# mitiko/weath3rb0i

Hardware: AMD Instinct MI355X
Metric: encode MiB/s, 64 KiB blocks, bit-exact vs CPU ref (higher is better)
Workload: dtype u32

## Files before the change

include/w3hip.h:

```cpp
#ifndef W3HIP_H
#define W3HIP_H

#include <stddef.h>
#include <stdint.h>

#ifdef __cplusplus
extern "C" {
#endif

#define W3_ABI_VERSION 8

enum {
    W3_OK            =  0,
    W3_E_INVALID     = -1,
    W3_E_NOSPACE     = -2,
    W3_E_HIP         = -3,
    W3_E_UNSUPPORTED = -4,
    W3_E_NOMEM       = -5,
    W3_E_FORMAT      = -6,
    W3_E_CORRUPT     = -7
};

enum { W3_NODE_ORDERN = 1, W3_NODE_BEST_OF_TWO = 2, W3_NODE_SLOT_STATE = 3, W3_NODE_APM = 4 };
enum { W3_HIST_NONE = 0, W3_HIST_RAW = 1, W3_HIST_AC = 2, W3_HIST_HUFF = 3 };
// ... 202 lines not shown
                       const uint8_t *in, size_t n, uint8_t *out, size_t out_cap, size_t *out_len);
int w3_decompress_stream(w3_ctx *ctx, const w3_model_spec *spec,
                         const uint8_t *in, size_t in_len, uint8_t *out, size_t out_cap, size_t *out_len);

int w3_predict_blocks(w3_ctx *ctx, const w3_model_spec *spec,
                      const uint8_t *in, size_t n, size_t block_size, uint16_t *p_out);

int w3_stationary_table(const uint8_t *buf, size_t n, uint16_t table[8]);

int w3_huff_tables(const uint8_t *buf, size_t n, uint8_t huff_size, uint8_t rem_huff_size, w3_huff_table *out);

#define W3_STAT_TILE 4096u
#define W3_STAT_BATCH 64u
#define W3_HIST_REP 16u
typedef struct w3_prep_profile {
    float hist_ms, hist_sum_ms, stat_count_ms, stat_walk_ms;
    uint32_t halvings[8];
    uint16_t table[8];
    uint64_t counts[256];
} w3_prep_profile;
int w3_histogram(w3_ctx *ctx, const uint8_t *in, size_t n, uint64_t counts[256]);
int w3_histogram_device(w3_ctx *ctx, const uint8_t *d_in, size_t n, uint64_t counts[256] , void *stream);
int w3_stationary_table_staged(w3_ctx *ctx, const uint8_t *in, size_t n, uint16_t table[8]);
int w3_stationary_table_device(w3_ctx *ctx, const uint8_t *d_in, size_t n, uint16_t table[8] , void *stream);
int w3_huff_code_from_counts(const uint64_t counts[256], uint8_t huffman_size, w3_huff_code *out);
int w3_huff_tables_from_counts(const uint64_t counts[256], uint8_t huff_size, uint8_t rem_huff_size, w3_huff_table *out);
int w3_table_prep_profile(w3_ctx *ctx, const uint8_t *d_in, size_t n, uint32_t hist_rep, w3_prep_profile *out);

#define W3_STATE_TABLE_SIZE 3963
int w3_state_table(uint16_t *out );
int w3_stretch_squash(int16_t *stretch , uint16_t *squash );

int w3_selftest_counter_p(w3_ctx *ctx, uint64_t *mismatches);

int w3_debug_get_stamps(w3_ctx *ctx, uint64_t out[8]);

typedef struct w3_timing {
    float    predict_ms;
    float    coder_ms;
    float    pack_ms;
    float    generic_ms;
    float    total_ms;
    uint32_t path;
    uint32_t n_coder_launches;
    uint64_t coder_bytes;
    uint64_t predict_bytes;
    uint32_t n_recoded_blocks;
    float    apm_ms;
    float    slot_ms;
    uint32_t n_slot_launches;
    float    achash_ms;
    uint32_t n_parts;
    uint32_t n_lds_faults;
    uint32_t n_wide;
    float    part_ms[4];
    float    rank_ms[4];
    float    small_ms;
} w3_timing;
int w3_get_timing(const w3_ctx *ctx, w3_timing *out);

#ifdef __cplusplus
}
#endif
#endif
```

weath3rb0i_amd/_lib.py:

```python
import ctypes as C
import os

HERE = os.path.dirname(os.path.abspath(__file__))
SO = os.environ.get("W3HIP_SO") or os.path.join(HERE, "libw3hip.so")

W3_MAX_NODES = 31
W3_NODE_ORDERN, W3_NODE_BEST_OF_TWO, W3_NODE_SLOT_STATE, W3_NODE_APM = 1, 2, 3, 4
W3_APM_ORDER0, W3_APM_ORDER1 = 0, 1
W3_MAX_APM = 4
W3_HIST_NONE, W3_HIST_RAW, W3_HIST_AC, W3_HIST_HUFF = 0, 1, 2, 3
W3_MAX_HUFF = 4
W3_OK, W3_E_INVALID, W3_E_NOSPACE, W3_E_HIP, W3_E_UNSUPPORTED, W3_E_NOMEM, W3_E_FORMAT = 0, -1, -2, -3, -4, -5, -6
W3_E_CORRUPT = -7
W3_OPT_PATH, W3_OPT_TIMING, W3_OPT_CODER, W3_OPT_ACC_LIMIT, W3_OPT_DEBUG_STAMPS, W3_OPT_VARIANT, W3_OPT_SLOT_BUDGET_MB, W3_OPT_VERIFY, W3_OPT_FAULT_BLOCK, W3_OPT_TUNE, W3_OPT_HOST_CHUNK_BLOCKS, W3_OPT_FAULT_KERNELS, W3_OPT_AOH_BATCH_BLOCKS = 1, 2, 3, 4, 5, 7, 8, 9, 10, 11, 12, 13, 14
W3_OPT_EXPORT_EPOCH = 15
W3_VAR_NO_LDS_ATOMICS, W3_VAR_PARTITION4, W3_VAR_NO_CHAINED_PARTITION, W3_VAR_CM_UNSTAGED, W3_VAR_NO_SIDE_STREAM, W3_VAR_INJECT_LDS_FAULT = 1, 2, 4, 8, 16, 32
W3_VAR_HALF_CU, W3_VAR_FULL_CU = 64, 128
W3_VAR_SLOT_TABLE, W3_VAR_SLOT_SORTED, W3_VAR_DECODE_LANE, W3_VAR_AOH_DECODE_SPEC = 256, 512, 1024, 2048
W3_GATHER_AUTO, W3_GATHER_RCCL, W3_GATHER_PEER_COPY = 0, 1, 2
W3_PATH_AUTO, W3_PATH_GENERIC, W3_PATH_TWOPHASE, W3_PATH_SPEC = 0, 1, 2, 3


class Node(C.Structure):
    _fields_ = [("kind", C.c_uint8), ("bits", C.c_uint8), ("align", C.c_uint8), ("history", C.c_uint8),
# ... 19 lines not shown
class Check(C.Structure):
    _fields_ = [("crc", C.c_void_p), ("bad_block", C.c_uint64), ("n_bad", C.c_uint64)]


class Timing(C.Structure):
    _fields_ = [("predict_ms", C.c_float), ("coder_ms", C.c_float), ("pack_ms", C.c_float), ("generic_ms", C.c_float),
                ("total_ms", C.c_float), ("path", C.c_uint32), ("n_coder_launches", C.c_uint32),
                ("coder_bytes", C.c_uint64), ("predict_bytes", C.c_uint64), ("n_recoded_blocks", C.c_uint32), ("apm_ms", C.c_float),
                ("slot_ms", C.c_float), ("n_slot_launches", C.c_uint32), ("achash_ms", C.c_float), ("n_parts", C.c_uint32),
                ("n_lds_faults", C.c_uint32), ("n_wide", C.c_uint32), ("part_ms", C.c_float * 4), ("rank_ms", C.c_float * 4),
                ("small_ms", C.c_float)]


class PrepProfile(C.Structure):
    _fields_ = [("hist_ms", C.c_float), ("hist_sum_ms", C.c_float), ("stat_count_ms", C.c_float), ("stat_walk_ms", C.c_float),
                ("halvings", C.c_uint32 * 8), ("table", C.c_uint16 * 8), ("counts", C.c_uint64 * 256)]


class ExportProfile(C.Structure):
    _fields_ = [("epochs", C.c_uint64), ("replays", C.c_uint64), ("halvings", C.c_uint64),
                ("count_ms", C.c_float), ("apply_ms", C.c_float), ("replay_ms", C.c_float), ("total_ms", C.c_float)]


class ExportEntropyProfile(C.Structure):
    _fields_ = [("base", ExportProfile), ("key_ms", C.c_float), ("huff_fixed_epochs", C.c_uint64)]


W3_STAT_TILE, W3_STAT_BATCH, W3_HIST_REP = 4096, 64, 16

EXPORTS = [
    "w3_abi_version", "w3_strerror", "w3_last_error", "w3_ctx_create", "w3_ctx_destroy", "w3_spec_validate",
    "w3_ctx_set_option", "w3_max_compressed_size", "w3_encode_blocks", "w3_decode_blocks", "w3_encode_blocks_device",
    "w3_decode_blocks_device", "w3_encode_submit", "w3_encode_wait", "w3_encode_max_in_flight", "w3_compress_stream", "w3_decompress_stream", "w3_predict_blocks", "w3_stationary_table",
    "w3_get_timing", "w3_selftest_counter_p", "w3_debug_get_stamps", "w3_state_table", "w3_stretch_squash", "w3_huff_tables",
    "w3_shard_range", "w3_encode_blocks_sharded", "w3_encode_blocks_sharded_device", "w3_encode_stats", "w3_encode_stats_device", "w3_sweep_ordern", "w3_sweep_ordern_device", "w3_export_counters",
    "w3_encode_host_submit", "w3_encode_host_wait", "w3_encode_host_max_in_flight", "w3_rccl_library", "w3_rccl_status",
    "w3_encode_sharded_submit", "w3_encode_sharded_wait", "w3_encode_sharded_max_in_flight",
    "w3_decode_ranges", "w3_decode_ranges_device",
    "w3_huff_code_table", "w3_aoh_max_compressed_size", "w3_aoh_encode_blocks", "w3_aoh_encode_blocks_device", "w3_aoh_decode_blocks",
    "w3_aoh_decode_blocks_device", "w3_aoh_encode_stats", "w3_aoh_encode_stats_device", "w3_sweep_ac_over_huffman",
    "w3_sweep_ac_over_huffman_device", "w3_aoh_decode_ranges", "w3_aoh_decode_ranges_device", "w3_aoh_decode_spec_covers",
    "w3_crc32_blocks", "w3_crc32_blocks_device", "w3_crc32_verify_device", "w3_decode_blocks_checked", "w3_decode_ranges_checked",
    "w3_decode_ranges_device_checked", "w3_aoh_decode_blocks_checked", "w3_aoh_decode_ranges_checked", "w3_aoh_decode_ranges_device_checked",
    "w3_histogram", "w3_histogram_device", "w3_stationary_table_staged", "w3_stationary_table_device", "w3_huff_code_from_counts",
    "w3_huff_tables_from_counts", "w3_table_prep_profile",
    "w3_export_counters_device", "w3_export_counters_staged", "w3_export_get_profile",
    "w3_export_entropy_device", "w3_export_entropy_staged", "w3_export_entropy_get_profile",
]

_lib = None


def load():
    global _lib
    if _lib is not None:
        return _lib
    if not os.path.exists(SO):
        raise ImportError(
            "weath3rb0i_amd: HIP extension %s is missing - run `python -m weath3rb0i_amd.build` "
            "(or __graft_entry__.build()).  There is no CPU fallback." % SO)
    try:
        import torch
    except ImportError:
        pass
    lib = C.CDLL(SO)
    vp, sz = C.c_void_p, C.c_size_t
    lib.w3_abi_version.restype = C.c_int
    lib.w3_strerror.restype = C.c_char_p
    lib.w3_strerror.argtypes = [C.c_int]
    lib.w3_last_error.restype = C.c_char_p
    lib.w3_last_error.argtypes = [vp]
    lib.w3_ctx_create.argtypes = [C.c_int, C.POINTER(vp)]
    lib.w3_ctx_destroy.argtypes = [vp]
    lib.w3_ctx_destroy.restype = None
    lib.w3_spec_validate.argtypes = [C.POINTER(ModelSpec)]
    lib.w3_ctx_set_option.argtypes = [vp, C.c_int, C.c_int64]
    lib.w3_max_compressed_size.restype = sz
    lib.w3_max_compressed_size.argtypes = [sz, sz]
    lib.w3_encode_blocks.argtypes = [vp, C.POINTER(ModelSpec), vp, sz, sz, vp, sz, C.POINTER(sz), vp]
    lib.w3_decode_blocks.argtypes = [vp, C.POINTER(ModelSpec), vp, sz, vp, sz, sz, C.c_uint64, vp]
    lib.w3_encode_blocks_device.argtypes = [vp, C.POINTER(ModelSpec), vp, sz, sz, vp, sz, vp, vp, vp]
    lib.w3_decode_blocks_device.argtypes = [vp, C.POINTER(ModelSpec), vp, sz, vp, sz, sz, C.c_uint64, vp, vp]
    lib.w3_encode_submit.argtypes = [vp, C.POINTER(ModelSpec), vp, sz, sz, vp, sz, vp, vp, vp, C.POINTER(C.c_int)]
    lib.w3_encode_wait.argtypes = [vp, C.c_int]
    lib.w3_encode_max_in_flight.argtypes = [C.POINTER(ModelSpec), sz, sz]
    lib.w3_encode_max_in_flight.restype = C.c_int
    lib.w3_compress_stream.argtypes = [vp, C.POINTER(ModelSpec), vp, sz, vp, sz, C.POINTER(sz)]
    lib.w3_decompress_stream.argtypes = [vp, C.POINTER(ModelSpec), vp, sz, vp, sz, C.POINTER(sz)]
    lib.w3_predict_blocks.argtypes = [vp, C.POINTER(ModelSpec), vp, sz, sz, vp]
    lib.w3_stationary_table.argtypes = [vp, sz, vp]
    lib.w3_selftest_counter_p.argtypes = [vp, C.POINTER(C.c_uint64)]
    lib.w3_debug_get_stamps.argtypes = [vp, C.POINTER(C.c_uint64 * 8)]
    lib.w3_get_timing.argtypes = [vp, C.POINTER(Timing)]
    lib.w3_state_table.argtypes = [vp]
    lib.w3_stretch_squash.argtypes = [vp, vp]
    lib.w3_huff_tables.argtypes = [vp, sz, C.c_uint8, C.c_uint8, C.POINTER(HuffTable)]
    lib.w3_shard_range.argtypes = [sz, C.c_int, C.c_int, C.POINTER(sz), C.POINTER(sz)]
    lib.w3_encode_blocks_sharded.argtypes = [C.POINTER(vp), C.c_int, C.POINTER(ModelSpec), vp, sz, sz, vp, sz, C.POINTER(sz), vp]
    lib.w3_encode_blocks_sharded_device.argtypes = [C.POINTER(vp), C.c_int, C.POINTER(ModelSpec), C.POINTER(vp), C.POINTER(sz), sz, C.c_int, vp, sz, vp,
                                                    C.POINTER(C.c_uint64), C.c_int]
    lib.w3_encode_stats.argtypes = [vp, C.POINTER(ModelSpec), vp, sz, sz, vp]
    lib.w3_encode_stats_device.argtypes = [vp, C.POINTER(ModelSpec), vp, sz, sz, vp, vp]
    lib.w3_sweep_ordern.argtypes = [vp, vp, sz, sz, vp, vp, sz, vp]
    lib.w3_sweep_ordern_device.argtypes = [vp, vp, sz, sz, vp, vp, sz, vp]
    lib.w3_export_counters.argtypes = [vp, C.POINTER(ModelSpec), vp, sz, vp]
    lib.w3_encode_host_submit.argtypes = [vp, C.POINTER(ModelSpec), vp, sz, sz, vp, sz, vp, C.POINTER(C.c_int)]
    lib.w3_encode_host_wait.argtypes = [vp, C.c_int, C.POINTER(sz)]
    lib.w3_encode_host_max_in_flight.argtypes = [C.POINTER(ModelSpec), sz, sz]
    lib.w3_encode_host_max_in_flight.restype = C.c_int
    lib.w3_encode_sharded_submit.argtypes = [C.POINTER(vp), C.c_int, C.POINTER(ModelSpec), C.POINTER(vp), C.POINTER(sz), sz, C.POINTER(C.c_int)]
    lib.w3_encode_sharded_wait.argtypes = [C.POINTER(vp), C.c_int, C.c_int, C.c_int, vp, sz, vp, C.POINTER(C.c_uint64), C.c_int]
    lib.w3_encode_sharded_max_in_flight.argtypes = [C.POINTER(ModelSpec), C.POINTER(sz), C.c_int, sz]
    lib.w3_encode_sharded_max_in_flight.restype = C.c_int
    lib.w3_decode_ranges.argtypes = [vp, C.POINTER(ModelSpec), vp, sz, vp, sz, sz, C.c_uint64, C.POINTER(Range), sz, vp, sz, C.POINTER(sz)]
    lib.w3_decode_ranges_device.argtypes = [vp, C.POINTER(ModelSpec), vp, sz, vp, sz, sz, C.c_uint64, C.POINTER(Range), sz, vp, sz, C.POINTER(sz), vp]
    hc, u8 = C.POINTER(HuffCode), C.c_uint8
    lib.w3_huff_code_table.argtypes = [vp, sz, u8, hc]
    lib.w3_aoh_max_compressed_size.restype = sz
    lib.w3_aoh_max_compressed_size.argtypes = [sz, sz, hc]
    lib.w3_aoh_encode_blocks.argtypes = [vp, hc, u8, vp, sz, sz, vp, sz, C.POINTER(sz), vp]
    lib.w3_aoh_encode_blocks_device.argtypes = [vp, hc, u8, vp, sz, sz, vp, sz, vp, vp, vp]
    lib.w3_aoh_decode_blocks.argtypes = [vp, hc, u8, vp, sz, vp, sz, sz, C.c_uint64, vp]
    lib.w3_aoh_decode_blocks_device.argtypes = [vp, hc, u8, vp, sz, vp, sz, sz, C.c_uint64, vp, vp]
    lib.w3_aoh_decode_ranges.argtypes = [vp, hc, u8, vp, sz, vp, sz, sz, C.c_uint64, C.POINTER(Range), sz, vp, sz, C.POINTER(sz)]
# ... 35 lines not shown
```

weath3rb0i_amd/csrc/w3_device.h:

```cpp
#pragma once
#include <hip/hip_runtime.h>
#include <stdint.h>

namespace w3 {

__device__ __forceinline__ uint32_t counter_p(uint32_t c0, uint32_t c1) {
    const uint32_t d = c0 + c1 + 2u;
    const uint32_t a = c1 + 1u;
    const float t = (float)a * __builtin_amdgcn_rcpf((float)d);
    uint32_t p = (uint32_t)__builtin_fmaf(t, 65536.0f, 0.47f);
    const uint32_t d2 = d + d;
    const uint32_t R = ((a << 17) + d) - __umul24(p, d2);
    return p + (R >= d2 ? 1u : 0u);
}

__device__ __forceinline__ uint32_t counter_p_packed(uint32_t c) { return counter_p(c & 0xFFFFu, c >> 16); }

__device__ __forceinline__ uint32_t counter_update_packed(uint32_t c, uint32_t bit) {
    uint32_t c0 = c & 0xFFFFu, c1 = c >> 16;
    if (bit) c1 += 1u; else c0 += 1u;
    if ((bit ? c1 : c0) == 0xFFFFu) {
        c0 = (c0 >> 1) + (c0 & 1u);
        c1 = (c1 >> 1) + (c1 & 1u);
    }
    return c0 | (c1 << 16);
}

__device__ __forceinline__ uint32_t opinion_dist(uint32_t p) { return p >= 32768u ? p - 32768u : 32768u - p; }
typedef unsigned short u16x2 __attribute__((ext_vector_type(2)));
typedef short i16x2 __attribute__((ext_vector_type(2)));
__device__ __forceinline__ u16x2 as_u16x2(uint32_t v) { return __builtin_bit_cast(u16x2, v); }
__device__ __forceinline__ i16x2 as_i16x2(u16x2 v) { return __builtin_bit_cast(i16x2, v); }
__device__ __forceinline__ uint32_t as_u32(u16x2 v) { return __builtin_bit_cast(uint32_t, v); }
__device__ __forceinline__ uint32_t as_u32(i16x2 v) { return __builtin_bit_cast(uint32_t, v); }
__device__ __forceinline__ u16x2 pk_opinion_dist(u16x2 p) {
    const u16x2 half = {32768, 32768};
    return __builtin_elementwise_max(p, half) - __builtin_elementwise_min(p, half);
}
__device__ __forceinline__ uint32_t pk_farther_mask(u16x2 d, u16x2 e) {
    uint32_t m;
    asm("v_pk_sub_i16 %0, %1, %2\n\tv_pk_ashrrev_i16 %0, 15, %0 op_sel_hi:[0,1]" : "=&v"(m) : "v"(as_u32(d)), "v"(as_u32(e)));
    return m;
}


struct BitSink {
    uint64_t acc;
    uint32_t nb;
    uint8_t *base;
// ... 237 lines not shown
```

weath3rb0i_amd/csrc/w3_predict.h:

```cpp
#pragma once
#include "w3_device.h"
#include "../../include/w3hip.h"

namespace w3 {

#define W3_PF 8

#define W3_HALF_CU_LDS 81920u
template <int NW, size_t USED> struct HalfCuPad { static constexpr size_t words = (NW > 1 && USED < W3_HALF_CU_LDS) ? (W3_HALF_CU_LDS - USED + 3u) / 4u : (NW > 1 ? 0u : 1u); };
template <size_t WORDS> struct HalfCuPadDecl {
    static __device__ __forceinline__ void keep(uint64_t n) {
        __shared__ uint32_t pad_[WORDS];
        if (n == ~0ull) pad_[threadIdx.x % WORDS] = 1u;
    }
};
template <> struct HalfCuPadDecl<0> { static __device__ __forceinline__ void keep(uint64_t) {} };
#define W3_HALF_CU_PAD(NW, USED) HalfCuPadDecl<((NW) > 1 ? HalfCuPad<NW, (USED)>::words : 0u)>::keep(a.n);

struct PredictArgs {
    const uint8_t *in;
    uint64_t n;
    uint32_t block_size, nblocks;
    uint4 *P;
    const uint2 *keys;
// ... 51 lines not shown
#pragma unroll
        for (int j = 0; j < 8; j++) {
            uint64_t m = ~0ull;
#pragma unroll
            for (int k = 0; k < H; k++) m &= X[8 - j + k];
            M[j] = m;
        }
    }
}

template <int H>
__device__ __forceinline__ void match_keys(uint2 k8, uint64_t M[8]) {
#pragma unroll
    for (int j = 0; j < 8; j++) {
        const uint32_t key = ((j < 4 ? k8.x : k8.y) >> (8 * (j & 3))) & 0xFFu;
        uint32_t mlo = 0xFFFFFFFFu, mhi = 0xFFFFFFFFu;
#pragma unroll
        for (int k = 0; k < H; k++) {
            const uint32_t sm = (uint32_t)__builtin_amdgcn_sbfe((int)key, k, 1);
            const uint64_t B = __ballot(sm != 0u);
            mlo &= ~((uint32_t)B ^ sm);
            mhi &= ~((uint32_t)(B >> 32) ^ sm);
        }
        M[j] = ((uint64_t)mhi << 32) | mlo;
    }
}

__device__ __forceinline__ uint32_t mbcnt64(uint64_t m) {
    return __builtin_amdgcn_mbcnt_hi((uint32_t)(m >> 32), __builtin_amdgcn_mbcnt_lo((uint32_t)m, 0u));
}

template <bool GROUPED>
__device__ __forceinline__ void rank_round(uint32_t c0, const uint32_t key[8], const uint64_t M[8], uint64_t seg, bool valid, bool rd,
                                           uint32_t *tbl, uint32_t p[8], uint32_t fin[8], uint32_t &wmask) {
    __asm__ volatile("" ::: "memory");
    const uint64_t gt = lane_gt_mask();
    const int lane = threadIdx.x & 63;
    wmask = 0u;
    uint32_t basev[8];
#pragma unroll
    for (int j = 0; j < 8; j++) basev[j] = tbl[j * 256 + key[j]];
#pragma unroll
    for (int j = 0; j < 8; j++) {
        const uint64_t Mj = M[j] & seg;
        const uint32_t bit = (c0 >> (7 - j)) & 1u;
        const uint64_t ones = __ballot(bit) & Mj;
        uint32_t base = basev[j];
        if constexpr (GROUPED) base = rd ? base : 0u;
        const uint32_t b0 = base & 0xFFFFu, b1 = base >> 16;
        const uint32_t n1l = mbcnt64(ones), n0l = mbcnt64(Mj) - n1l;
        uint32_t s0 = b0 + n0l, s1 = b1 + n1l;
        const bool last = valid && (Mj & gt) == 0ull;
        uint32_t f0 = s0 + (bit ^ 1u), f1 = s1 + bit;
        uint64_t satm = __ballot(last && (f0 >= 65535u || f1 >= 65535u));
        uint32_t f = f0 | (f1 << 16);
        while (satm) {
            const int k = __ffsll((long long)satm) - 1;
            const uint64_t Mc = readlane_u64(Mj, k);
            const uint64_t Oc = readlane_u64(ones, k);
            uint32_t st = readlane_u32(base, k);
            uint64_t it = Mc;
            while (it) {
                const int m = __ffsll((long long)it) - 1;
                it &= it - 1;
                if (lane == m) { s0 = st & 0xFFFFu; s1 = st >> 16; }
                st = counter_update_packed(st, (uint32_t)(Oc >> m) & 1u);
            }
            if (lane == k) f = st;
            satm &= satm - 1;
        }
        p[j] = counter_p(s0, s1);
        fin[j] = f;
        wmask |= last ? (1u << j) : 0u;
    }
    if constexpr (!GROUPED) {
#pragma unroll
        for (int j = 0; j < 8; j++)
            if ((wmask >> j) & 1u) tbl[j * 256 + key[j]] = fin[j];
        __asm__ volatile("" ::: "memory");
    }
}

#define W3_ATOMIC_LIM 65400u
#ifndef W3_ATOMIC_MAXSEG
#define W3_ATOMIC_MAXSEG 4u
#endif
typedef uint16_t w3_u16x2 __attribute__((ext_vector_type(2)));

__device__ __forceinline__ void atomic_round(uint32_t *tbl, uint32_t c0, const uint32_t key[8], bool on, uint32_t v[8]) {
#pragma unroll
    for (int j = 0; j < 8; j++) {
        const uint32_t inc = on ? (((c0 >> (7 - j)) & 1u) ? 0x10000u : 1u) : 0u;
        v[j] = __hip_atomic_fetch_add(&tbl[j * 256 + key[j]], inc, __ATOMIC_RELAXED, __HIP_MEMORY_SCOPE_WORKGROUP);
    }
}
__device__ __forceinline__ bool atomic_round_hot(const uint32_t v[8]) {
    w3_u16x2 m = __builtin_bit_cast(w3_u16x2, v[0]);
#pragma unroll
    for (int j = 1; j < 8; j++) m = __builtin_elementwise_max(m, __builtin_bit_cast(w3_u16x2, v[j]));
    return __ballot(max((uint32_t)m.x, (uint32_t)m.y) >= W3_ATOMIC_LIM) != 0ull;
}

__host__ __device__ __forceinline__ uint32_t lds_order_hash(uint32_t wave, uint32_t round, uint32_t lane) {
    uint32_t x = (wave * 64u + round) * 64u + lane + 0x9E3779B9u;
    x ^= x >> 16; x *= 0x7FEB352Du; x ^= x >> 15; x *= 0x846CA68Bu; x ^= x >> 16;
    return x;
}
__host__ __device__ __forceinline__ uint32_t lds_order_key(uint32_t wave, uint32_t h) {
    const uint32_t kind = wave & 3u;
    return kind == 0 ? 77u : kind == 1 ? (h & 7u) * 32u + 1u : kind == 2 ? (h & 255u) : (h & 2047u);
}
__global__ void __launch_bounds__(64) k_lds_order_selftest(uint32_t *old) {
    __shared__ uint32_t tbl[2048];
    const uint32_t lane = threadIdx.x;
    for (uint32_t i = lane; i < 2048u; i += 64u) tbl[i] = 0u;
    __builtin_amdgcn_wave_barrier();
    for (uint32_t r = 0; r < 32u; r++) {
        const uint32_t h = lds_order_hash(blockIdx.x, r, lane);
        old[(blockIdx.x * 32u + r) * 64u + lane] =
            __hip_atomic_fetch_add(&tbl[lds_order_key(blockIdx.x, h)], (h >> 20) & 1u ? 0x10000u : 1u, __ATOMIC_RELAXED, __HIP_MEMORY_SCOPE_WORKGROUP);
    }
}

__device__ __forceinline__ uint4 pack_p(const uint32_t p[8]) {
    return make_uint4(p[0] | (p[1] << 16), p[2] | (p[3] << 16), p[4] | (p[5] << 16), p[6] | (p[7] << 16));
}

__device__ __forceinline__ uint32_t mix_pair(uint32_t cur, uint32_t nw) {
    const uint32_t c_lo = cur & 0xFFFFu, c_hi = cur >> 16, n_lo = nw & 0xFFFFu, n_hi = nw >> 16;
    const uint32_t lo = opinion_dist(n_lo) > opinion_dist(c_lo) ? n_lo : c_lo;
    const uint32_t hi = opinion_dist(n_hi) > opinion_dist(c_hi) ? n_hi : c_hi;
    return lo | (hi << 16);
}
__device__ __forceinline__ uint4 mix_p(uint4 cur, uint4 nw) {
    return make_uint4(mix_pair(cur.x, nw.x), mix_pair(cur.y, nw.y), mix_pair(cur.z, nw.z), mix_pair(cur.w, nw.w));
}

#define W3_HD __host__ __device__ __forceinline__
#include "w3_verify.h"
#undef W3_HD
#include "w3_window.h"

template <int H, bool KEYS, int NW = 1>
__global__ void __launch_bounds__(64 * NW) k_predict_small(PredictArgs a) {
    __shared__ uint32_t tbl_[NW][8 * 256];
    __shared__ uint32_t st_w_[NW][W3_PF * 64];
    __shared__ uint2 st_k_[NW][KEYS ? W3_PF * 64 : 1];
    W3_HALF_CU_PAD(NW, sizeof(tbl_) + sizeof(st_w_) + sizeof(st_k_))
    const int lane = threadIdx.x & 63;
    const uint32_t wv = threadIdx.x >> 6;
    uint32_t *tbl = tbl_[wv], *st_w = st_w_[wv];
    uint2 *st_k = st_k_[wv];
    constexpr uint32_t KM = (1u << H) - 1u;
    for (uint32_t b = blockIdx.x * NW + wv; b < a.nblocks; b += gridDim.x * NW) {
        const uint64_t off = (uint64_t)b * a.block_size;
        const uint32_t len = (uint32_t)((a.n - off) < a.block_size ? (a.n - off) : a.block_size);
        const uint8_t *blk = a.in + off;
#pragma unroll
        for (int k = 0; k < 32; k++) tbl[k * 64 + lane] = 0u;
        __builtin_amdgcn_wave_barrier();
        bool exact = (a.dbg_flags & 2u) != 0u;
        const uint32_t first = window_head(off, 3u);
        const uint32_t last = len - 1u;
        uint32_t nw[W3_PF]; uint2 nk[W3_PF];
#pragma unroll
        for (int r = 0; r < W3_PF; r++) {
            const uint32_t ic = min((uint32_t)(r * 64 + lane), last);
            if constexpr (KEYS) { nk[r] = a.keys[off + ic]; nw[r] = blk[ic]; } else { nw[r] = load_window(blk, ic, first); nk[r] = make_uint2(0, 0); }
        }
        for (uint32_t bbase = 0; bbase < len; bbase += 64u * W3_PF) {
            __asm__ volatile("" ::: "memory");
            __builtin_amdgcn_wave_barrier();
#pragma unroll
            for (int r = 0; r < W3_PF; r++) { st_w[r * 64 + lane] = nw[r]; if constexpr (KEYS) st_k[r * 64 + lane] = nk[r]; }
            __asm__ volatile("" ::: "memory");
            __builtin_amdgcn_wave_barrier();
#pragma unroll
            for (int r = 0; r < W3_PF; r++) {
                const uint32_t ic = min(bbase + (uint32_t)((W3_PF + r) * 64 + lane), last);
                if constexpr (KEYS) { nk[r] = a.keys[off + ic]; nw[r] = blk[ic]; } else nw[r] = load_window(blk, ic, first);
            }
#pragma unroll 1
          for (uint32_t rr = 0; rr < W3_PF; rr++) {
            const uint32_t base = bbase + rr * 64u;
            if (base >= len) break;
            const uint32_t i = base + lane;
            const bool valid = i < len;
            const uint32_t w = st_w[rr * 64u + lane];
            uint2 k8 = make_uint2(0, 0);
            if constexpr (KEYS) k8 = st_k[rr * 64u + lane];
            uint32_t c0 = 0, key[8], p[8];
            if constexpr (KEYS) {
                c0 = valid ? w : 0u;
#pragma unroll
                for (int j = 0; j < 8; j++) key[j] = ((j < 4 ? k8.x : k8.y) >> (8 * (j & 3))) & KM;
            } else {
                const uint32_t wv = valid ? w : 0u;
                c0 = wv & 0xFFu;
#pragma unroll
                for (int j = 0; j < 8; j++) key[j] = ((wv & 0xFFFFu) >> (8 - j)) & KM;
            }
            if (!exact) {
                uint32_t v[8];
                __asm__ volatile("" ::: "memory");
                atomic_round(tbl, c0, key, valid, v);
                __asm__ volatile("" ::: "memory");
                if ((a.dbg_flags & 8u) && base == 64u && (a.fault_block == 0xFFFFFFFFu || a.fault_block == b)) v[0] = (uint32_t)__shfl_xor((int)v[0], 1, 64);
#pragma unroll
                for (int j = 0; j < 8; j++) p[j] = counter_p_packed(v[j]);
                exact = atomic_round_hot(v);
            } else {
                uint64_t M[8];
                if constexpr (KEYS) match_keys<H>(valid ? k8 : make_uint2(0, 0), M);
                else match_windows<H>((valid ? w : 0u) & 0xFFFFu, M);
                const uint64_t seg = __ballot(valid);
                uint32_t fin[8], wm;
                rank_round<false>(c0, key, M, seg, valid, true, tbl, p, fin, wm);
            }
            {
                uint4 *dst = valid ? a.P + (off + i) : a.sink + lane;
                *dst = pack_p(p);
            }
          }
        }
    }
}

__device__ __forceinline__ uint32_t wave_excl_scan_u32(uint32_t v, uint32_t *total) {
    const int lane = threadIdx.x & 63;
    uint32_t inc = v;
#pragma unroll
    for (int d = 1; d < 64; d <<= 1) {
        uint32_t o = __shfl_up(inc, d, 64);
        if (lane >= d) inc += o;
    }
    *total = __shfl(inc, 63, 64);
    return inc - v;
}


template <int NPASS, bool C2ONLY = false>
__device__ __forceinline__ void partition_hist(const uint8_t *blk, uint32_t len, uint32_t first, uint32_t *hist) {
    const int lane = threadIdx.x & 63;
// ... 385 lines not shown
                }
            }
        }
        if (lane == 0) found = 0u;
        sp[lane] = found;
        if (lane == 0) sp[W3_SLICES] = len;
        W3_STAMP(4);
        if (a.dbg && lane == 0) atomicAdd(&a.dbg[6], 1ull);
    }
}

template <int NBYTES, int NW = 1, int PF = W3_PF, bool FAULT = false>
__global__ void __launch_bounds__(64 * NW) k_rank_sorted(PredictArgs a) {
    __shared__ uint32_t tbl_[NW][8 * 256];
    __shared__ uint2 st_r_[NW][PF * 64];
    W3_HALF_CU_PAD(NW, sizeof(tbl_) + sizeof(st_r_))
    const int lane = threadIdx.x & 63;
    uint32_t *tbl = tbl_[threadIdx.x >> 6];
    uint2 *st_r = st_r_[threadIdx.x >> 6];
    const uint32_t njobs = a.nblocks * W3_SLICES;
    for (;;) {
        uint32_t job = 0;
        if (lane == 0) job = atomicAdd(a.job_counter, 1u);
        job = __builtin_amdgcn_readfirstlane(job);
        if (job >= njobs) break;
        const uint32_t b = job / W3_SLICES, sl = job % W3_SLICES;
        const uint64_t off = (uint64_t)b * a.block_size;
        const uint32_t *sp = a.splits + (uint64_t)b * (W3_SLICES + 1u);
        const uint32_t lo = sp[sl], hi = sp[sl + 1];
        if (lo >= hi) continue;
        const uint32_t len = hi - lo;
        const uint2 *perm = a.rec + off + lo;
        unsigned long long t_prev = a.dbg ? __builtin_amdgcn_s_memtime() : 0ull;
#pragma unroll
        for (int k = 0; k < 32; k++) tbl[k * 64 + lane] = 0u;
        __builtin_amdgcn_wave_barrier();
        bool exact = (a.dbg_flags & 2u) != 0u;
        bool dirty = false;
        uint32_t open_g = 0xFFFFFFFFu;
        const uint32_t last = len - 1u;
        uint2 rn[PF];
#pragma unroll
        for (int r = 0; r < PF; r++) rn[r] = perm[min((uint32_t)(r * 64 + lane), last)];
        for (uint32_t bbase = 0; bbase < len; bbase += 64u * (uint32_t)PF) {
            __asm__ volatile("" ::: "memory");
            __builtin_amdgcn_wave_barrier();
#pragma unroll
            for (int r = 0; r < PF; r++) st_r[r * 64 + lane] = rn[r];
            __asm__ volatile("" ::: "memory");
            __builtin_amdgcn_wave_barrier();
#pragma unroll
            for (int r = 0; r < PF; r++) rn[r] = perm[min(bbase + (uint32_t)((PF + r) * 64 + lane), last)];
#pragma unroll 1
          for (uint32_t rr = 0; rr < (uint32_t)PF; rr++) {
            const uint32_t base = bbase + rr * 64u;
            if (base >= len) break;
            const uint32_t e = base + lane;
            const bool valid = e < len;
            const uint2 r_c = st_r[rr * 64u + lane];
            const uint32_t i = r_c.x; const uint32_t w = valid ? r_c.y : 0u;
            const uint32_t c0 = w & 0xFFu;
            const uint32_t g = NBYTES == 1 ? ((w >> 8) & 0xFFu) : ((w >> 8) & 0xFFFFu);
            const uint32_t ck = NBYTES == 1 ? ((w >> 16) & 0xFFu) : (w >> 24);
            const uint32_t w16 = (ck << 8) | c0;
            uint32_t gprev = __shfl_up(g, 1, 64);
            if (lane == 0) gprev = open_g;
            const uint64_t vm = __ballot(valid);
            const uint64_t heads = __ballot(valid && g != gprev) | 1ull;
            const uint64_t hle = heads & (lane_lt_mask() | (1ull << lane));
            const int start = 63 - __clzll((long long)hle);
            const uint64_t hgt = heads & lane_gt_mask();
            const uint64_t below_end = hgt ? ((1ull << (__ffsll((long long)hgt) - 1)) - 1ull) : ~0ull;
            const uint64_t seg = below_end & ~((1ull << start) - 1ull) & vm;
            uint32_t key[8], p[8];
#pragma unroll
            for (int j = 0; j < 8; j++) key[j] = (w16 >> (8 - j)) & 0xFFu;
            uint32_t *vt = tbl;
            const int lastlane = 63 - __clzll((long long)vm);
            const uint32_t g_last = readlane_u32(g, lastlane);
            uint64_t hm = heads & vm;
            if (!exact && (uint32_t)__popcll(hm) <= a.maxseg) {
                uint32_t v[8];
#pragma unroll
                for (int j = 0; j < 8; j++) v[j] = 0u;
                __asm__ volatile("" ::: "memory");
                if (dirty && readlane_u32(g, 0) != open_g) {
#pragma unroll
                    for (int k = 0; k < 32; k++) vt[k * 64 + lane] = 0u;
                    dirty = false;
                }
                bool carried = dirty;
                while (hm) {
                    const int st = __ffsll((long long)hm) - 1;
                    hm &= hm - 1ull;
                    const int en = hm ? __ffsll((long long)hm) - 1 : 64;
                    const bool in = valid && lane >= st && lane < en;
                    __asm__ volatile("" ::: "memory");
                    if (in) atomic_round(vt, c0, key, true, v);
                    __asm__ volatile("" ::: "memory");
                    if (hm) {
                        if (carried) {
#pragma unroll
                            for (int k = 0; k < 32; k++) vt[k * 64 + lane] = 0u;
                        } else if (in) {
#pragma unroll
                            for (int j = 0; j < 8; j++) vt[j * 256 + key[j]] = 0u;
                        }
                    }
                    carried = false;
                }
                __asm__ volatile("" ::: "memory");
                if constexpr (FAULT) {
                    if (64u - (lo + base) < 64u && (a.fault_block == 0xFFFFFFFFu || a.fault_block == b)) v[0] = (uint32_t)__shfl_xor((int)v[0], 1, 64);
                }
#pragma unroll
                for (int j = 0; j < 8; j++) p[j] = counter_p_packed(v[j]);
                exact = atomic_round_hot(v);
            } else {
                uint32_t fin[8], wm;
                uint64_t M[8];
                match_windows<8>(w16, M);
                rank_round<true>(c0, key, M, seg, valid, g == open_g, vt, p, fin, wm);
                if (g_last != open_g && dirty) {
#pragma unroll
                    for (int k = 0; k < 32; k++) vt[k * 64 + lane] = 0u;
                    dirty = false;
                }
                __builtin_amdgcn_wave_barrier();
                if (valid && g == g_last) {
#pragma unroll
                    for (int j = 0; j < 8; j++)
                        if ((wm >> j) & 1u) vt[j * 256 + key[j]] = fin[j];
                }
                __asm__ volatile("" ::: "memory");
                __builtin_amdgcn_wave_barrier();
            }
            dirty = true;
            open_g = g_last;
            {
                uint4 *dst = (valid && !(a.dbg_flags & 1u)) ? a.P + (off + ((a.dbg_flags & 4u) ? (i & 0xFFFu) : i)) : a.sink + lane;
                *dst = pack_p(p);
            }
          }
        }
        W3_STAMP(3);
        if (a.dbg && lane == 0 && sl == 0) atomicAdd(&a.dbg[7], 1ull);
    }
}

#define W3_HUFF_WALK 40u
struct HuffKeyArgs { const uint8_t *in; uint64_t n; uint32_t block_size; uint32_t hmask; const w3_huff_table *tb; uint2 *keys;
                     uint32_t *redo;
                     uint32_t nblocks;
                     uint32_t *keys32;  };

__device__ __forceinline__ void huff_hashes_of(uint32_t cb, uint32_t c0, const uint16_t *rcode, const uint8_t *rlen, uint32_t (&h)[8]) {
#pragma unroll
    for (int j = 0; j < 8; j++) {
// ... 192 lines not shown
```

weath3rb0i_amd/csrc/w3_selftest.h:

```cpp
#pragma once
#include "w3_device.h"

namespace w3 {
__global__ void __launch_bounds__(256) k_selftest_counter_p(unsigned long long *mismatches, uint32_t c0_lo, uint32_t c0_hi) {
    const uint64_t total = (uint64_t)(c0_hi - c0_lo) << 16;
    unsigned long long bad = 0;
    for (uint64_t i = (uint64_t)blockIdx.x * blockDim.x + threadIdx.x; i < total; i += (uint64_t)gridDim.x * blockDim.x) {
        const uint32_t c0 = c0_lo + (uint32_t)(i >> 16), c1 = (uint32_t)(i & 0xFFFFu);
        const uint64_t p = ((uint64_t)1 << 17) * ((uint64_t)c1 + 1) / ((uint64_t)c0 + c1 + 2);
        const uint32_t want = (uint32_t)((p >> 1) + (p & 1));
        if (counter_p(c0, c1) != want) bad++;
    }
    if (bad) atomicAdd(mismatches, bad);
}
}
```

weath3rb0i_amd/csrc/w3hip.hip:

```cpp
#include "../../include/w3hip.h"

#include <hip/hip_runtime.h>

#include <algorithm>
#include <cstddef>
#include <cstdio>
#include <cstring>
#include <mutex>
#include <string>
#include <thread>
#include <vector>

#include "w3_spec.h"
#include "w3_huff.h"
#include "w3_generic.h"
#include "w3_cm.h"
#include "w3_decode_spec.h"
#include "w3_pack.h"
#include "w3_tables_plan.h"
#include "w3_jobs.h"
#include "w3_twophase.h"
#include "w3_selftest.h"
#include "w3_sweep.h"
#include "w3_aoh.h"
// ... 3380 lines not shown
    HIPCHK(ctx, hipStreamSynchronize(s));
    HIPCHK(ctx, hipMemcpy(p_out, d_p, n * 16, hipMemcpyDeviceToHost));
    return W3_OK;
}

extern "C" int w3_state_table(uint16_t *out) {
    if (!out) return W3_E_INVALID;
    std::vector<StEntry> t(kStSize);
    build_state_table(t.data());
    for (int i = 0; i < kStSize; i++) { out[3 * i] = t[i].prob; out[3 * i + 1] = t[i].next0; out[3 * i + 2] = t[i].next1; }
    return W3_OK;
}

extern "C" int w3_stretch_squash(int16_t *stretch, uint16_t *squash) {
    if (!stretch || !squash) return W3_E_INVALID;
    build_stretch_squash(stretch, squash);
    return W3_OK;
}

extern "C" int w3_selftest_counter_p(w3_ctx *ctx, uint64_t *mismatches) {
    if (!ctx || !mismatches) return W3_E_INVALID;
    HIPCHK(ctx, hipSetDevice(ctx->device));
    ENSURE(ctx, ctx->total, 8);
    HIPCHK(ctx, hipMemsetAsync(ctx->total.p, 0, 8, ctx->stream));
    for (uint32_t lo = 0; lo < 65536; lo += 4096) {
        hipLaunchKernelGGL(k_selftest_counter_p, dim3(256 * 16), dim3(256), 0, ctx->stream, (unsigned long long *)ctx->total.p, lo, lo + 4096);
        HIPCHK(ctx, hipGetLastError());
    }
    HIPCHK(ctx, hipMemcpyAsync(mismatches, ctx->total.p, 8, hipMemcpyDeviceToHost, ctx->stream));
    HIPCHK(ctx, hipStreamSynchronize(ctx->stream));
    return W3_OK;
}

extern "C" int w3_debug_get_stamps(w3_ctx *ctx, uint64_t out[8]) {
    if (!ctx || !out) return W3_E_INVALID;
    memset(out, 0, 64);
    if (!ctx->jobs[0].tp.dbg) return W3_OK;
    HIPCHK(ctx, hipSetDevice(ctx->device));
    HIPCHK(ctx, hipDeviceSynchronize());
    HIPCHK(ctx, hipMemcpy(out, ctx->jobs[0].tp.dbg, 64, hipMemcpyDeviceToHost));
    return W3_OK;
}
```

Baseline: 14090.

## Store biased counters in LDS and compute rounded probability via packed float reciprocal

Counters in the LDS tables now start at a bias so each entry directly holds (denominator, numerator) instead of (c0, c1). The probability can then be computed with a float reciprocal, an FMA and an integer correction in place of the exact counter_p division. Other changes: hot-counter detection only runs when the base position could reach the limit, window keys come from a single 24-bit multiply, the single-segment case skips the segmented atomic loop, and packing uses v_perm. Leaving the fast path means unbiasing the whole table, and a new selftest checks the approximate rounding against the exact formula.

```diff
diff --git a/include/w3hip.h b/include/w3hip.h
--- a/include/w3hip.h
+++ b/include/w3hip.h
@@ -258,6 +258,7 @@
 int w3_stretch_squash(int16_t *stretch , uint16_t *squash );
 
 int w3_selftest_counter_p(w3_ctx *ctx, uint64_t *mismatches);
+int w3_selftest_counter_p_round(w3_ctx *ctx, uint64_t *mismatches);
 
 int w3_debug_get_stamps(w3_ctx *ctx, uint64_t out[8]);
 
diff --git a/weath3rb0i_amd/_lib.py b/weath3rb0i_amd/_lib.py
--- a/weath3rb0i_amd/_lib.py
+++ b/weath3rb0i_amd/_lib.py
@@ -75,7 +75,7 @@
     "w3_abi_version", "w3_strerror", "w3_last_error", "w3_ctx_create", "w3_ctx_destroy", "w3_spec_validate",
     "w3_ctx_set_option", "w3_max_compressed_size", "w3_encode_blocks", "w3_decode_blocks", "w3_encode_blocks_device",
     "w3_decode_blocks_device", "w3_encode_submit", "w3_encode_wait", "w3_encode_max_in_flight", "w3_compress_stream", "w3_decompress_stream", "w3_predict_blocks", "w3_stationary_table",
-    "w3_get_timing", "w3_selftest_counter_p", "w3_debug_get_stamps", "w3_state_table", "w3_stretch_squash", "w3_huff_tables",
+    "w3_get_timing", "w3_selftest_counter_p", "w3_selftest_counter_p_round", "w3_debug_get_stamps", "w3_state_table", "w3_stretch_squash", "w3_huff_tables",
     "w3_shard_range", "w3_encode_blocks_sharded", "w3_encode_blocks_sharded_device", "w3_encode_stats", "w3_encode_stats_device", "w3_sweep_ordern", "w3_sweep_ordern_device", "w3_export_counters",
     "w3_encode_host_submit", "w3_encode_host_wait", "w3_encode_host_max_in_flight", "w3_rccl_library", "w3_rccl_status",
     "w3_encode_sharded_submit", "w3_encode_sharded_wait", "w3_encode_sharded_max_in_flight",
@@ -133,6 +133,7 @@
     lib.w3_predict_blocks.argtypes = [vp, C.POINTER(ModelSpec), vp, sz, sz, vp]
     lib.w3_stationary_table.argtypes = [vp, sz, vp]
     lib.w3_selftest_counter_p.argtypes = [vp, C.POINTER(C.c_uint64)]
+    lib.w3_selftest_counter_p_round.argtypes = [vp, C.POINTER(C.c_uint64)]
     lib.w3_debug_get_stamps.argtypes = [vp, C.POINTER(C.c_uint64 * 8)]
     lib.w3_get_timing.argtypes = [vp, C.POINTER(Timing)]
     lib.w3_state_table.argtypes = [vp]
diff --git a/weath3rb0i_amd/csrc/w3_device.h b/weath3rb0i_amd/csrc/w3_device.h
--- a/weath3rb0i_amd/csrc/w3_device.h
+++ b/weath3rb0i_amd/csrc/w3_device.h
@@ -15,6 +15,30 @@
 }
 
 __device__ __forceinline__ uint32_t counter_p_packed(uint32_t c) { return counter_p(c & 0xFFFFu, c >> 16); }
+
+#define W3_CTR_BIAS 0x00010002u
+typedef float f32x2 __attribute__((ext_vector_type(2)));
+__device__ __forceinline__ void counter_p_round2_parts(f32x2 fa, f32x2 fd, const uint32_t d[2], const uint32_t w[2], uint32_t p[2]) {
+    const f32x2 r = {__builtin_amdgcn_rcpf(fd.x), __builtin_amdgcn_rcpf(fd.y)};
+    const f32x2 x = __builtin_elementwise_fma(fa * r, (f32x2)(-65536.0f), (f32x2)(-1.47f));
+    const int m[2] = {(int)x.x, (int)x.y};
+#pragma unroll
+    for (int k = 0; k < 2; k++) {
+        const int Q = __mul24(m[k], (int)d[k]) + (int)w[k];
+        asm("v_cmp_lt_i32 vcc, %1, %2\n\tv_subb_co_u32 %0, vcc, 0, %3, vcc" : "=v"(p[k]) : "v"(Q), "v"((int)d[k] - Q), "v"(m[k]) : "vcc");
+    }
+}
+__device__ __forceinline__ void counter_p_round2(uint32_t W0, uint32_t W1, uint32_t p[2]) {
+    const uint32_t d[2] = {W0 & 0xFFFFu, W1 & 0xFFFFu}, w[2] = {W0, W1};
+    const f32x2 fa = {(float)(W0 >> 16), (float)(W1 >> 16)}, fd = {(float)d[0], (float)d[1]};
+    counter_p_round2_parts(fa, fd, d, w, p);
+}
+__device__ __forceinline__ void counter_p_round8(const uint32_t W[8], uint32_t p[8]) {
+#pragma unroll
+    for (int j = 0; j < 8; j += 2) counter_p_round2(W[j], W[j + 1], p + j);
+}
+__device__ __forceinline__ uint32_t counter_unbias(uint32_t W) { return W - 0x10001u - (W >> 16); }
+__device__ __forceinline__ uint32_t counter_bias(uint32_t c) { return c + W3_CTR_BIAS + (c >> 16); }
 
 __device__ __forceinline__ uint32_t counter_update_packed(uint32_t c, uint32_t bit) {
     uint32_t c0 = c & 0xFFFFu, c1 = c >> 16;
diff --git a/weath3rb0i_amd/csrc/w3_predict.h b/weath3rb0i_amd/csrc/w3_predict.h
--- a/weath3rb0i_amd/csrc/w3_predict.h
+++ b/weath3rb0i_amd/csrc/w3_predict.h
@@ -107,7 +107,7 @@
 
 template <bool GROUPED>
 __device__ __forceinline__ void rank_round(uint32_t c0, const uint32_t key[8], const uint64_t M[8], uint64_t seg, bool valid, bool rd,
-                                           uint32_t *tbl, uint32_t p[8], uint32_t fin[8], uint32_t &wmask) {
+                                           uint32_t *tbl, uint32_t p[8], uint32_t fin[8], uint32_t &wmask, bool biased = false) {
     __asm__ volatile("" ::: "memory");
     const uint64_t gt = lane_gt_mask();
     const int lane = threadIdx.x & 63;
@@ -120,7 +120,7 @@
         const uint64_t Mj = M[j] & seg;
         const uint32_t bit = (c0 >> (7 - j)) & 1u;
         const uint64_t ones = __ballot(bit) & Mj;
-        uint32_t base = basev[j];
+        uint32_t base = biased ? counter_unbias(basev[j]) : basev[j];
         if constexpr (GROUPED) base = rd ? base : 0u;
         const uint32_t b0 = base & 0xFFFFu, b1 = base >> 16;
         const uint32_t n1l = mbcnt64(ones), n0l = mbcnt64(Mj) - n1l;
@@ -145,7 +145,7 @@
             satm &= satm - 1;
         }
         p[j] = counter_p(s0, s1);
-        fin[j] = f;
+        fin[j] = biased ? counter_bias(f) : f;
         wmask |= last ? (1u << j) : 0u;
     }
     if constexpr (!GROUPED) {
@@ -162,18 +162,37 @@
 #endif
 typedef uint16_t w3_u16x2 __attribute__((ext_vector_type(2)));
 
-__device__ __forceinline__ void atomic_round(uint32_t *tbl, uint32_t c0, const uint32_t key[8], bool on, uint32_t v[8]) {
-#pragma unroll
-    for (int j = 0; j < 8; j++) {
-        const uint32_t inc = on ? (((c0 >> (7 - j)) & 1u) ? 0x10000u : 1u) : 0u;
-        v[j] = __hip_atomic_fetch_add(&tbl[j * 256 + key[j]], inc, __ATOMIC_RELAXED, __HIP_MEMORY_SCOPE_WORKGROUP);
-    }
-}
+__device__ __forceinline__ void window_keys8(uint32_t w16, uint32_t key[8]) {
+#pragma unroll
+    for (int j = 0; j < 8; j += 2) {
+        const uint32_t y = __umul24(w16 & 0xFFFFu, (1u << j) + (1u << (17 + j)));
+        key[j] = (y >> 8) & 0xFFu;
+        key[j + 1] = y >> 24;
+    }
+}
+__device__ __forceinline__ void atomic_round_incs(uint32_t c0, bool on, uint32_t inc[8]) {
+#pragma unroll
+    for (int j = 0; j < 8; j++) inc[j] = (((c0 >> (7 - j)) & 1u) << 16) | (on ? 1u : 0u);
+}
+__device__ __forceinline__ void atomic_round(uint32_t *tbl, const uint32_t inc[8], const uint32_t key[8], uint32_t v[8]) {
+#pragma unroll
+    for (int j = 0; j < 8; j++)
+        v[j] = __hip_atomic_fetch_add(&tbl[j * 256 + key[j]], inc[j], __ATOMIC_RELAXED, __HIP_MEMORY_SCOPE_WORKGROUP);
+}
+__device__ __forceinline__ bool atomic_round_may_be_hot(uint32_t base) { return base + 63u >= W3_ATOMIC_LIM; }
 __device__ __forceinline__ bool atomic_round_hot(const uint32_t v[8]) {
     w3_u16x2 m = __builtin_bit_cast(w3_u16x2, v[0]);
 #pragma unroll
     for (int j = 1; j < 8; j++) m = __builtin_elementwise_max(m, __builtin_bit_cast(w3_u16x2, v[j]));
-    return __ballot(max((uint32_t)m.x, (uint32_t)m.y) >= W3_ATOMIC_LIM) != 0ull;
+    return __ballot((uint32_t)m.x >= W3_ATOMIC_LIM) != 0ull;
+}
+__device__ __forceinline__ void table_unbias(uint32_t *tbl, int lane) {
+    __asm__ volatile("" ::: "memory");
+    __builtin_amdgcn_wave_barrier();
+#pragma unroll
+    for (int k = 0; k < 32; k++) tbl[k * 64 + lane] = counter_unbias(tbl[k * 64 + lane]);
+    __asm__ volatile("" ::: "memory");
+    __builtin_amdgcn_wave_barrier();
 }
 
 __host__ __device__ __forceinline__ uint32_t lds_order_hash(uint32_t wave, uint32_t round, uint32_t lane) {
@@ -197,8 +216,9 @@
     }
 }
 
+__device__ __forceinline__ uint32_t pack_p2(uint32_t lo, uint32_t hi) { return __builtin_amdgcn_perm(hi, lo, 0x05040100u); }
 __device__ __forceinline__ uint4 pack_p(const uint32_t p[8]) {
-    return make_uint4(p[0] | (p[1] << 16), p[2] | (p[3] << 16), p[4] | (p[5] << 16), p[6] | (p[7] << 16));
+    return make_uint4(pack_p2(p[0], p[1]), pack_p2(p[2], p[3]), pack_p2(p[4], p[5]), pack_p2(p[6], p[7]));
 }
 
 __device__ __forceinline__ uint32_t mix_pair(uint32_t cur, uint32_t nw) {
@@ -231,10 +251,11 @@
         const uint64_t off = (uint64_t)b * a.block_size;
         const uint32_t len = (uint32_t)((a.n - off) < a.block_size ? (a.n - off) : a.block_size);
         const uint8_t *blk = a.in + off;
-#pragma unroll
-        for (int k = 0; k < 32; k++) tbl[k * 64 + lane] = 0u;
+        bool exact = (a.dbg_flags & 2u) != 0u;
+        const uint32_t empty = exact ? 0u : W3_CTR_BIAS;
+#pragma unroll
+        for (int k = 0; k < 32; k++) tbl[k * 64 + lane] = empty;
         __builtin_amdgcn_wave_barrier();
-        bool exact = (a.dbg_flags & 2u) != 0u;
         const uint32_t first = window_head(off, 3u);
         const uint32_t last = len - 1u;
         uint32_t nw[W3_PF]; uint2 nk[W3_PF];
@@ -272,18 +293,21 @@
             } else {
                 const uint32_t wv = valid ? w : 0u;
                 c0 = wv & 0xFFu;
-#pragma unroll
-                for (int j = 0; j < 8; j++) key[j] = ((wv & 0xFFFFu) >> (8 - j)) & KM;
+                if constexpr (H == 8) window_keys8(wv, key);
+                else {
+#pragma unroll
+                    for (int j = 0; j < 8; j++) key[j] = ((wv & 0xFFFFu) >> (8 - j)) & KM;
+                }
             }
             if (!exact) {
-                uint32_t v[8];
-                __asm__ volatile("" ::: "memory");
-                atomic_round(tbl, c0, key, valid, v);
+                uint32_t v[8], inc[8];
+                atomic_round_incs(c0, valid, inc);
+                __asm__ volatile("" ::: "memory");
+                atomic_round(tbl, inc, key, v);
                 __asm__ volatile("" ::: "memory");
                 if ((a.dbg_flags & 8u) && base == 64u && (a.fault_block == 0xFFFFFFFFu || a.fault_block == b)) v[0] = (uint32_t)__shfl_xor((int)v[0], 1, 64);
-#pragma unroll
-                for (int j = 0; j < 8; j++) p[j] = counter_p_packed(v[j]);
-                exact = atomic_round_hot(v);
+                counter_p_round8(v, p);
+                if (atomic_round_may_be_hot(base) && atomic_round_hot(v)) { exact = true; table_unbias(tbl, lane); }
             } else {
                 uint64_t M[8];
                 if constexpr (KEYS) match_keys<H>(valid ? k8 : make_uint2(0, 0), M);
@@ -735,10 +759,13 @@
         const uint32_t len = hi - lo;
         const uint2 *perm = a.rec + off + lo;
         unsigned long long t_prev = a.dbg ? __builtin_amdgcn_s_memtime() : 0ull;
-#pragma unroll
-        for (int k = 0; k < 32; k++) tbl[k * 64 + lane] = 0u;
+        bool exact = (a.dbg_flags & 2u) != 0u;
+        {
+            const uint32_t empty = exact ? 0u : W3_CTR_BIAS;
+#pragma unroll
+            for (int k = 0; k < 32; k++) tbl[k * 64 + lane] = empty;
+        }
         __builtin_amdgcn_wave_barrier();
-        bool exact = (a.dbg_flags & 2u) != 0u;
         bool dirty = false;
         uint32_t open_g = 0xFFFFFFFFu;
         const uint32_t last = len - 1u;
@@ -776,57 +803,63 @@
             const uint64_t below_end = hgt ? ((1ull << (__ffsll((long long)hgt) - 1)) - 1ull) : ~0ull;
             const uint64_t seg = below_end & ~((1ull << start) - 1ull) & vm;
             uint32_t key[8], p[8];
-#pragma unroll
-            for (int j = 0; j < 8; j++) key[j] = (w16 >> (8 - j)) & 0xFFu;
+            window_keys8(w16, key);
             uint32_t *vt = tbl;
             const int lastlane = 63 - __clzll((long long)vm);
             const uint32_t g_last = readlane_u32(g, lastlane);
             uint64_t hm = heads & vm;
             if (!exact && (uint32_t)__popcll(hm) <= a.maxseg) {
-                uint32_t v[8];
-#pragma unroll
-                for (int j = 0; j < 8; j++) v[j] = 0u;
+                uint32_t v[8], inc[8];
                 __asm__ volatile("" ::: "memory");
                 if (dirty && readlane_u32(g, 0) != open_g) {
 #pragma unroll
-                    for (int k = 0; k < 32; k++) vt[k * 64 + lane] = 0u;
+                    for (int k = 0; k < 32; k++) vt[k * 64 + lane] = W3_CTR_BIAS;
                     dirty = false;
                 }
-                bool carried = dirty;
-                while (hm) {
-                    const int st = __ffsll((long long)hm) - 1;
-                    hm &= hm - 1ull;
-                    const int en = hm ? __ffsll((long long)hm) - 1 : 64;
-                    const bool in = valid && lane >= st && lane < en;
+                if (hm == 1ull) {
+                    atomic_round_incs(c0, valid, inc);
                     __asm__ volatile("" ::: "memory");
-                    if (in) atomic_round(vt, c0, key, true, v);
-                    __asm__ volatile("" ::: "memory");
-                    if (hm) {
-                        if (carried) {
-#pragma unroll
-                            for (int k = 0; k < 32; k++) vt[k * 64 + lane] = 0u;
-                        } else if (in) {
-#pragma unroll
-                            for (int j = 0; j < 8; j++) vt[j * 256 + key[j]] = 0u;
+                    atomic_round(vt, inc, key, v);
+                } else {
+                    atomic_round_incs(c0, true, inc);
+#pragma unroll
+                    for (int j = 0; j < 8; j++) v[j] = W3_CTR_BIAS;
+                    bool carried = dirty;
+                    while (hm) {
+                        const int st = __ffsll((long long)hm) - 1;
+                        hm &= hm - 1ull;
+                        const int en = hm ? __ffsll((long long)hm) - 1 : 64;
+                        const bool in = valid && lane >= st && lane < en;
+                        __asm__ volatile("" ::: "memory");
+                        if (in) atomic_round(vt, inc, key, v);
+                        __asm__ volatile("" ::: "memory");
+                        if (hm) {
+                            if (carried) {
+#pragma unroll
+                                for (int k = 0; k < 32; k++) vt[k * 64 + lane] = W3_CTR_BIAS;
+                            } else if (in) {
+#pragma unroll
+                                for (int j = 0; j < 8; j++) vt[j * 256 + key[j]] = W3_CTR_BIAS;
+                            }
                         }
+                        carried = false;
                     }
-                    carried = false;
                 }
                 __asm__ volatile("" ::: "memory");
                 if constexpr (FAULT) {
                     if (64u - (lo + base) < 64u && (a.fault_block == 0xFFFFFFFFu || a.fault_block == b)) v[0] = (uint32_t)__shfl_xor((int)v[0], 1, 64);
                 }
-#pragma unroll
-                for (int j = 0; j < 8; j++) p[j] = counter_p_packed(v[j]);
-                exact = atomic_round_hot(v);
+                counter_p_round8(v, p);
+                if (atomic_round_may_be_hot(base) && atomic_round_hot(v)) { exact = true; table_unbias(vt, lane); }
             } else {
                 uint32_t fin[8], wm;
                 uint64_t M[8];
                 match_windows<8>(w16, M);
-                rank_round<true>(c0, key, M, seg, valid, g == open_g, vt, p, fin, wm);
+                rank_round<true>(c0, key, M, seg, valid, g == open_g, vt, p, fin, wm, !exact);
                 if (g_last != open_g && dirty) {
-#pragma unroll
-                    for (int k = 0; k < 32; k++) vt[k * 64 + lane] = 0u;
+                    const uint32_t empty = exact ? 0u : W3_CTR_BIAS;
+#pragma unroll
+                    for (int k = 0; k < 32; k++) vt[k * 64 + lane] = empty;
                     dirty = false;
                 }
                 __builtin_amdgcn_wave_barrier();
diff --git a/weath3rb0i_amd/csrc/w3_selftest.h b/weath3rb0i_amd/csrc/w3_selftest.h
--- a/weath3rb0i_amd/csrc/w3_selftest.h
+++ b/weath3rb0i_amd/csrc/w3_selftest.h
@@ -13,4 +13,27 @@
     }
     if (bad) atomicAdd(mismatches, bad);
 }
+
+__global__ void __launch_bounds__(256) k_selftest_counter_p_round(unsigned long long *mismatches, uint32_t c0_lo, uint32_t c0_hi) {
+    const uint64_t total = (uint64_t)(c0_hi - c0_lo) << 16;
+    unsigned long long bad = 0;
+    for (uint64_t i = (uint64_t)blockIdx.x * blockDim.x + threadIdx.x; i < total; i += (uint64_t)gridDim.x * blockDim.x) {
+        const uint32_t c0 = c0_lo + (uint32_t)(i >> 16), c1 = (uint32_t)(i & 0xFFFFu);
+        const uint64_t p = ((uint64_t)1 << 17) * ((uint64_t)c1 + 1) / ((uint64_t)c0 + c1 + 2);
+        const uint32_t want = (uint32_t)((p >> 1) + (p & 1));
+        const uint32_t d = c0 + c1 + 2u, a = c1 + 1u;
+        uint32_t got[2];
+        if (d <= 65535u) {
+            const uint32_t W = counter_bias(c0 | (c1 << 16));
+            counter_p_round2(W, W, got);
+            if (W != (d | (a << 16)) || counter_unbias(W) != (c0 | (c1 << 16))) got[0] = 0xFFFFFFFFu;
+        } else {
+            const uint32_t dd[2] = {d, d}, ww[2] = {d + (a << 16), d + (a << 16)};
+            const f32x2 fa = {(float)a, (float)a}, fd = {(float)d, (float)d};
+            counter_p_round2_parts(fa, fd, dd, ww, got);
+        }
+        if (got[0] != want || got[1] != want) bad++;
+    }
+    if (bad) atomicAdd(mismatches, bad);
 }
+}
diff --git a/weath3rb0i_amd/csrc/w3hip.hip b/weath3rb0i_amd/csrc/w3hip.hip
--- a/weath3rb0i_amd/csrc/w3hip.hip
+++ b/weath3rb0i_amd/csrc/w3hip.hip
@@ -3436,6 +3436,20 @@
     return W3_OK;
 }
 
+extern "C" int w3_selftest_counter_p_round(w3_ctx *ctx, uint64_t *mismatches) {
+    if (!ctx || !mismatches) return W3_E_INVALID;
+    HIPCHK(ctx, hipSetDevice(ctx->device));
+    ENSURE(ctx, ctx->total, 8);
+    HIPCHK(ctx, hipMemsetAsync(ctx->total.p, 0, 8, ctx->stream));
+    for (uint32_t lo = 0; lo < 65536; lo += 4096) {
+        hipLaunchKernelGGL(k_selftest_counter_p_round, dim3(256 * 16), dim3(256), 0, ctx->stream, (unsigned long long *)ctx->total.p, lo, lo + 4096);
+        HIPCHK(ctx, hipGetLastError());
+    }
+    HIPCHK(ctx, hipMemcpyAsync(mismatches, ctx->total.p, 8, hipMemcpyDeviceToHost, ctx->stream));
+    HIPCHK(ctx, hipStreamSynchronize(ctx->stream));
+    return W3_OK;
+}
+
 extern "C" int w3_debug_get_stamps(w3_ctx *ctx, uint64_t out[8]) {
     if (!ctx || !out) return W3_E_INVALID;
     memset(out, 0, 64);
```

Result: no change. 14180, median of 6 (+0.6%).
